# al8n/serf

Hardware: NVIDIA H100
Metric: gossip edge-updates/sec @10M nodes (higher is better)
Workload: dtype u32

## Files before the change

serf_b200/csrc/serfsim.cu:

```cuda
#include <algorithm>
#include <cmath>
#include <cstdio>
#include <cstdlib>
#include <cstring>
#include <string>
#include <unordered_set>
#include <vector>

#include "../../include/serfsim.h"
#include "tick_kernel.cuh"
#include "wire.cuh"

using namespace sfs;

namespace {

thread_local std::string g_err;

int fail(int code, const std::string& msg) { g_err = msg; return code; }

#define CU(call)                                                                              \
  do {                                                                                        \
    cudaError_t e_ = (call);                                                                  \
    if (e_ != cudaSuccess)                                                                    \
// ... 130 lines not shown
  u64* d_grow = nullptr;
  bool gate_on = false;
  u32 gate_first = 0;
  std::vector<u32> launch_log;
  u32 launch_log_first = 0;
  cudaStream_t stream = nullptr;
  cudaEvent_t ev0 = nullptr, ev1 = nullptr;
  bool timing_open = false;
  double last_ms = 0.0;
  u64 last_launches = 0, launches = 0;
  serfsim_event_cb cb = nullptr;
  void* cb_user = nullptr;
  std::vector<u8> reported;
  int grid = 1;
  int ctas_per_sm = 4;
  u64* d_win_data[2] = {nullptr, nullptr};
  u32* d_ctrl = nullptr;
  u32* d_send_count = nullptr;
  u64** d_peer_data[2] = {nullptr, nullptr};
  u32** d_peer_ctrl = nullptr;
  u32 xepoch = 0;
  u32 win_cap = 0;
  u32 win_cap_base = 0;
  bool connected = false;
  bool loopback = false;
  serfsim_barrier_fn barrier = nullptr; serfsim_allreduce_u64_fn allreduce = nullptr; void* comm_user = nullptr;
  std::vector<void*> ipc_opened;
  bool tick_timing = false;
  size_t l2_persist_max = 0, l2_window_max = 0;
  bool l2_window = false;
  bool no_skip = false;
  bool compact = true;
  bool dedup = true;
  struct ResBuf { unsigned char* d = nullptr; cudaEvent_t copied = nullptr; bool used = false; };
  ResBuf res[4];
  u32 res_next = 0;
  cudaStream_t copy_stream = nullptr;
  cudaEvent_t ev_extracted = nullptr;
  std::vector<cudaEvent_t> tick_ev;
  std::vector<cudaEvent_t> mid_ev;
};

namespace {

int slot_of(const serfsim* h, u32 node) {
  for (u32 s = 0; s < h->R; ++s) if (h->subj[s] == node) return (int)s;
  return -1;
}

int ensure_trace(serfsim* h, u32 need) {
  if (need <= h->trace_cap) return 0;
  u32 cap = std::max<u32>(1024, h->trace_cap);
  while (cap < need) cap *= 2;
  u64* nt = nullptr; u32* nk = nullptr; u64* ng = nullptr;
  const bool sharded = h->cfg.world_size > 1;
  CU(cudaMalloc(&nt, (size_t)cap * 8 * sizeof(u64)));
  CU(cudaMalloc(&nk, ((size_t)cap + 1) * 4 * sizeof(u32)));
  CU(cudaMemsetAsync(nt, 0, (size_t)cap * 8 * sizeof(u64), h->stream));
  CU(cudaMemsetAsync(nk, 0, ((size_t)cap + 1) * 4 * sizeof(u32), h->stream));
  if (sharded) { CU(cudaMalloc(&ng, (size_t)cap * 8 * sizeof(u64))); CU(cudaMemsetAsync(ng, 0, (size_t)cap * 8 * sizeof(u64), h->stream)); }
  if (h->d_trace) {
    CU(cudaMemcpyAsync(nt, h->d_trace, (size_t)h->trace_cap * 8 * sizeof(u64), cudaMemcpyDeviceToDevice, h->stream));
    CU(cudaMemcpyAsync(nk, h->d_kinds, ((size_t)h->trace_cap + 1) * 4 * sizeof(u32), cudaMemcpyDeviceToDevice, h->stream));
    if (sharded) CU(cudaMemcpyAsync(ng, h->d_grow, (size_t)h->trace_cap * 8 * sizeof(u64), cudaMemcpyDeviceToDevice, h->stream));
    CU(cudaStreamSynchronize(h->stream));
    cudaFree(h->d_trace); cudaFree(h->d_kinds); cudaFree(h->d_grow);
// ... 43 lines not shown
    const u32 t = h->tick;
    const u64 launches_before = h->last_launches;
    auto lo = std::lower_bound(h->ops.begin(), h->ops.end(), t, [](const HostOp& o, u32 tt) { return o.tick < tt; });
    auto hi = std::upper_bound(h->ops.begin(), h->ops.end(), t, [](u32 tt, const HostOp& o) { return tt < o.tick; });
    const u32 eb = (u32)(lo - h->ops.begin()), ee = (u32)(hi - h->ops.begin());
    for (auto it = lo; it != hi; ++it) {
      const int s = slot_of(h, it->node);
      if (s >= 0) { if (it->op == SERFSIM_OP_FAIL) h->up_mask &= ~(1u << s); if (it->op == SERFSIM_OP_REJOIN) h->up_mask |= (1u << s); }
    }
    if (ee > eb) { launch_mark_events(h->d_busy, h->d_hot[(t & 1) ^ 1], h->d_ev_node, eb, ee, h->first, h->count, h->stream); h->last_launches++; }
    TickParams p{};
    p.n_local = h->count; p.first = h->first; p.n_global = h->N; p.R = h->R;
    p.fanout = h->cfg.fanout; p.probe_every = h->cfg.probe_interval_ticks; p.tick = t;
    p.down_mask = (~h->up_mask) & ((1u << h->R) - 1);
    h->ever_down |= p.down_mask;
    p.seed_lo = (u32)h->cfg.seed; p.seed_hi = (u32)(h->cfg.seed >> 32); p.ev_begin = eb; p.ev_end = ee;
    p.rules = h->rules;
    for (u32 s = 0; s < h->R; ++s) p.subj[s] = h->subj[s];
    p.rec = h->d_rec; p.qword = h->d_qword; p.inbox_rd = h->d_inbox[(t & 1) ^ 1]; p.inbox_wr = h->d_inbox[t & 1];
    p.node_state = h->d_node; p.busy = h->d_busy; p.watch = h->d_watch; p.row_ptr = h->d_rowptr; p.col = h->d_col;
    p.ev_node = h->d_ev_node; p.ev_op = h->d_ev_op; p.ev_slot = h->d_ev_slot;
    p.row = h->d_trace + (size_t)t * 8;
    p.kinds_prev = h->d_kinds + (size_t)t * 4;
    p.kinds_cur = h->d_kinds + ((size_t)t + 1) * 4;
    p.overflow = h->d_overflow;
    p.hot_rd = h->d_hot[(t & 1) ^ 1]; p.hot_wr = h->d_hot[t & 1];
    p.stage_col_bytes = h->stage_col_bytes;
    p.reap_now = (h->cfg.reap_interval_ticks && ((t + 1) % h->cfg.reap_interval_ticks) == 0) ? 1u : 0u;
    p.tombstone_ticks = h->cfg.tombstone_timeout_ticks; p.reconnect_ticks = h->cfg.reconnect_timeout_ticks; p.intent_ticks = h->cfg.recent_intent_timeout_ticks;
    p.stride = h->stride; p.n_tiles = h->n_tiles; p.tiles_per_cta = (h->n_tiles + h->grid - 1) / h->grid;
    p.force_all = (h->cfg.trace != 0) || h->no_skip || p.reap_now;
    p.compact = h->compact ? 1u : 0u;
    p.dedup = h->dedup ? 1u : 0u;
    p.udeg = h->udeg; p.ahead = h->ahead;
    p.tile_due = h->d_tile_due; p.node_due = h->d_node_due; p.hot_static = h->d_hot_static; p.sched = h->d_sched;
    p.sleep_on = (h->no_skip || h->byz_on) ? 0u : 1u;
    p.pp_every = (u32)std::max(0, h->cfg.push_pull_interval_ticks); p.reap_every = h->cfg.reap_interval_ticks;
    p.host_idle_until = h->d_pin_ctl + 2;
    const u32 xpar = h->xepoch & 1;
    p.world = (u32)h->cfg.world_size; p.rank = (u32)h->cfg.rank; p.shard_size = h->shard_size; p.win_cap = h->win_cap;
    p.win_data = h->d_peer_data[xpar]; p.send_count = h->d_send_count;
    p.peer_ctrl = h->d_peer_ctrl; p.stamp = h->xepoch + 1; p.xpar = xpar; p.loopback = h->loopback ? 1u : 0u;
    p.fuse_publish = (sharded && !h->byz_on && !getenv("SERFSIM_NO_FUSE")) ? 1u : 0u;
    p.shard_inv = (u32)(0x100000000ull / h->shard_size); p.xcap = p.world > 1 ? 392u / (p.world - 1) : 0u;
    Gate gate{};
    if (h->gate_on) {
      gate.ctl = h->d_runctl; gate.host_ctl = h->d_pin_ctl; gate.prev_row = t > h->gate_first ? grow + (size_t)(t - 1) * 8 : nullptr; gate.tick = t;
      gate.future_ops = (t > 0 && future_ops(h, t - 1)) ? 1u : 0u;
      gate.pp = (u32)std::max(0, h->cfg.push_pull_interval_ticks); gate.byz_on = h->byz_on ? 1u : 0u;
    }
    const u32* gate_word = h->gate_on ? h->d_runctl : nullptr;
    p.gate = gate; p.gate.evaluate = h->ue_table.n ? 0u : 1u;
    if (h->tick_timing) {
      while (h->tick_ev.size() < 2 * ((size_t)t + 1)) { cudaEvent_t e; CU(cudaEventCreate(&e)); h->tick_ev.push_back(e); }
      CU(cudaEventRecord(h->tick_ev[2 * (size_t)t], h->stream));
    }
    if (h->l2_window && h->l2_window_max) {
      cudaStreamAttrValue av{};
      const size_t bytes = (size_t)3 * h->R * h->stride * sizeof(u32);
      av.accessPolicyWindow.base_ptr = h->d_inbox[t & 1];
      av.accessPolicyWindow.num_bytes = std::min(bytes, h->l2_window_max);
      av.accessPolicyWindow.hitRatio = (float)std::min(1.0, (double)h->l2_persist_max / (double)std::max<size_t>(1, av.accessPolicyWindow.num_bytes));
      av.accessPolicyWindow.hitProp = cudaAccessPropertyPersisting;
      av.accessPolicyWindow.missProp = cudaAccessPropertyStreaming;
      CU(cudaStreamSetAttribute(h->stream, cudaStreamAttributeAccessPolicyWindow, &av));
    }
// ... 394 lines not shown
  CUB(cudaMalloc(&h->d_subj, MAX_SLOTS * 4)); CUB(cudaMalloc(&h->d_scratch, 64 * 8));
  CUB(cudaMalloc(&h->d_stage, (size_t)h->count * 8));
  CUB(cudaMalloc(&h->d_runctl, 2 * sizeof(u32)));
  CUB(cudaMemset(h->d_runctl, 0, 2 * sizeof(u32)));
  CUB(cudaHostAlloc(&h->pin_ctl, 4 * sizeof(u32), cudaHostAllocMapped));
  CUB(cudaHostGetDevicePointer(&h->d_pin_ctl, h->pin_ctl, 0));
  h->pin_ctl[0] = h->pin_ctl[1] = h->pin_ctl[2] = h->pin_ctl[3] = 0;
  CUB(cudaMalloc(&h->d_ones, 16));
  const u32 ones[4] = {0x40000000u, 0x40000000u, 0x40000000u, 1u};
  CUB(cudaMemcpy(h->d_ones, ones, 16, cudaMemcpyHostToDevice));
  CUB(cudaMemcpy(h->d_subj, h->subj.data(), h->R * 4, cudaMemcpyHostToDevice));
  {
    const char* e = getenv("SERFSIM_MINB");
    h->ctas_per_sm = (h->R == 1) ? ((e && atoi(e) == 5) ? 5 : (cfg->world_size > 1 ? tick_ctas_per_sm_r1s() : tick_ctas_per_sm_r1())) : tick_ctas_per_sm_rn();
  }
  h->grid = tick_grid_size(h->count, h->ctas_per_sm);
  h->grid_sv = tick_grid_size(h->count, cfg->world_size > 1 ? tick_ctas_per_sm_r1s() : tick_ctas_per_sm_r1());
  {
    int max_persist = 0, max_window = 0;
    cudaDeviceGetAttribute(&max_persist, cudaDevAttrMaxPersistingL2CacheSize, dev);
    cudaDeviceGetAttribute(&max_window, cudaDevAttrMaxAccessPolicyWindowSize, dev);
    h->l2_persist_max = (size_t)max_persist; h->l2_window_max = (size_t)max_window;
    int want = 0;
    if (const char* e = getenv("SERFSIM_L2_PERSIST")) want = atoi(e);
    if (want && max_persist > 0) cudaDeviceSetLimit(cudaLimitPersistingL2CacheSize, (size_t)max_persist);
    if (const char* e = getenv("SERFSIM_L2_WINDOW")) h->l2_window = atoi(e) != 0;
    if (getenv("SERFSIM_VERBOSE")) fprintf(stderr, "serfsim: L2 persisting max %d B, window max %d B, persist %d window %d\n", max_persist, max_window, want, (int)h->l2_window);
  }
  if (const char* e = getenv("SERFSIM_NO_SKIP")) h->no_skip = atoi(e) != 0;
  if (const char* e = getenv("SERFSIM_COMPACT")) h->compact = atoi(e) != 0;
  if (const char* e = getenv("SERFSIM_DEDUP")) h->dedup = atoi(e) != 0;
  if (const char* e = getenv("SERFSIM_AHEAD")) h->ahead = (u32)std::min(2, std::max(0, atoi(e)));
  if (const char* e = getenv("SERFSIM_SV")) h->sv = (u32)std::min(2, std::max(0, atoi(e)));
  if (cfg->world_size > 1) {
    if (cfg->world_size > 8) return bail(fail(SERFSIM_E_INVAL, "world_size > 8"));
    double factor = 1.25;
    if (const char* e = getenv("SERFSIM_WIN_FACTOR")) factor = atof(e);
    const double pad = (double)std::max(tick_grid_size(h->count, h->ctas_per_sm), h->grid_sv) * 8.0 * 160.0;
    double cap = (double)h->shard_size * cfg->fanout * h->R * 3.0 * factor / cfg->world_size + 4096.0 + pad;
    h->win_cap = (u32)std::min(cap, 4.0e9);
    h->win_cap_base = h->win_cap;
    for (int par = 0; par < 2; ++par) {
      CUB(cudaMalloc(&h->d_win_data[par], (size_t)cfg->world_size * h->win_cap * 8));
      CUB(cudaMemset(h->d_win_data[par], 0, (size_t)cfg->world_size * h->win_cap * 8));
      CUB(cudaMalloc(&h->d_peer_data[par], sizeof(u64*) * 8));
    }
    CUB(cudaMalloc(&h->d_ctrl, CTRL_BYTES));
    CUB(cudaMemset(h->d_ctrl, 0, CTRL_BYTES));
    CUB(cudaMalloc(&h->d_send_count, 8 * sizeof(u32)));
    CUB(cudaMemset(h->d_send_count, 0, 8 * sizeof(u32)));
    CUB(cudaMalloc(&h->d_peer_ctrl, sizeof(u32*) * 8));
    CUB(cudaMalloc(&h->d_anomaly, h->stride)); CUB(cudaMemset(h->d_anomaly, 0, h->stride));
    CUB(cudaMalloc(&h->d_byz_totals, 4 * 8)); CUB(cudaMemset(h->d_byz_totals, 0, 4 * 8));
    CUB(cudaMalloc(&h->d_peer_anomaly, sizeof(void*) * 8));
    if (cfg->push_pull_interval_ticks > 0) {
      CUB(cudaMalloc(&h->d_snap_rec, (size_t)h->R * h->stride * 32));
      CUB(cudaMalloc(&h->d_snap_node, (size_t)h->stride * 8));
      CUB(cudaMalloc(&h->d_peer_snap_rec, sizeof(void*) * 8));
      CUB(cudaMalloc(&h->d_peer_snap_node, sizeof(void*) * 8));
    }
  }
  {
    int rc = ensure_trace(h, 1024);
    if (rc) return bail(rc);
    rc = do_reset(h, cfg->seed);
    if (rc) return bail(rc);
// ... 652 lines not shown
```

serf_b200/csrc/tick_kernel.cu:

```cuda
#include <cstdlib>

#include "tick_kernel.cuh"
#include "byz.cuh"

namespace sfs {

namespace {

constexpr int BLOCK = 256;
#ifndef SFS_MB_R1
#define SFS_MB_R1 3
#endif
#ifndef SFS_MB_R1S
#define SFS_MB_R1S SFS_MB_R1
#endif
#ifndef SFS_MB_RN
#define SFS_MB_RN 1
#endif
constexpr u32 TILE_SHIFT = 8;
constexpr u32 MAX_TILES_PER_CTA = 1024;
static_assert((1u << TILE_SHIFT) == BLOCK, "tile = block");

struct Words { u32 w[8]; };

// ... 2 lines not shown
__device__ __forceinline__ u64 policy_evict_last() { u64 p; asm volatile("createpolicy.fractional.L2::evict_last.b64 %0, 1.0;" : "=l"(p)); return p; }

__device__ __forceinline__ Words ld_rec256(const uint4* ptr, u64 pol) {
  Words r;
  asm volatile("ld.global.L1::no_allocate.L2::cache_hint.v4.u32 {%0,%1,%2,%3}, [%8], %9;\n\t"
               "ld.global.L1::no_allocate.L2::cache_hint.v4.u32 {%4,%5,%6,%7}, [%8+16], %9;"
               : "=r"(r.w[0]), "=r"(r.w[1]), "=r"(r.w[2]), "=r"(r.w[3]), "=r"(r.w[4]), "=r"(r.w[5]), "=r"(r.w[6]), "=r"(r.w[7])
               : "l"(ptr), "l"(pol));
  return r;
}
__device__ __forceinline__ void st_rec256(uint4* ptr, const Words& r, u64 pol) {
  asm volatile("st.global.L2::cache_hint.v4.u32 [%0], {%1,%2,%3,%4}, %9;\n\t"
               "st.global.L2::cache_hint.v4.u32 [%0+16], {%5,%6,%7,%8}, %9;"
               :: "l"(ptr), "r"(r.w[0]), "r"(r.w[1]), "r"(r.w[2]), "r"(r.w[3]), "r"(r.w[4]), "r"(r.w[5]), "r"(r.w[6]), "r"(r.w[7]), "l"(pol) : "memory");
}
__device__ __forceinline__ u64 ld_u64_stream(const u64* ptr, u64 pol) {
  u64 v; asm volatile("ld.global.L1::no_allocate.L2::cache_hint.u64 %0, [%1], %2;" : "=l"(v) : "l"(ptr), "l"(pol)); return v;
}
__device__ __forceinline__ u32 ld_u32_stream(const u32* ptr, u64 pol) {
  u32 v; asm volatile("ld.global.L1::no_allocate.L2::cache_hint.u32 %0, [%1], %2;" : "=r"(v) : "l"(ptr), "l"(pol)); return v;
}
__device__ __forceinline__ void st_u32_stream(u32* ptr, u32 v, u64 pol) {
  asm volatile("st.global.L2::cache_hint.u32 [%0], %1, %2;" :: "l"(ptr), "r"(v), "l"(pol) : "memory");
}
__device__ __forceinline__ void st_u64_stream(u64* ptr, u64 v, u64 pol) {
  asm volatile("st.global.L2::cache_hint.u64 [%0], %1, %2;" :: "l"(ptr), "l"(v), "l"(pol) : "memory");
}
__device__ __forceinline__ void red_max_resident(u32* ptr, u32 v, u64 pol) {
  asm volatile("red.relaxed.gpu.global.max.L2::cache_hint.u32 [%0], %1, %2;" :: "l"(ptr), "r"(v), "l"(pol) : "memory");
}
__device__ __forceinline__ u32 peek_inbox(const u32* ptr, u64 pol) {
  u32 v; asm volatile("ld.global.L1::no_allocate.L2::cache_hint.u32 %0, [%1], %2;" : "=r"(v) : "l"(ptr), "l"(pol)); return v;
}
__device__ __forceinline__ void st_release_sys(u32* ptr, u32 v) { asm volatile("st.release.sys.global.u32 [%0], %1;" :: "l"(ptr), "r"(v) : "memory"); }
__device__ __forceinline__ u32 ld_acquire_sys(const u32* ptr) { u32 f; asm volatile("ld.acquire.sys.global.u32 %0, [%1];" : "=r"(f) : "l"(ptr) : "memory"); return f; }
#else
inline u64 policy_evict_first() { return 0; }
inline u64 policy_evict_last() { return 0; }
inline Words ld_rec256(const uint4* ptr, u64) { emu::probes[8] += 32; Words r; const u32* q = reinterpret_cast<const u32*>(ptr); for (int i = 0; i < 8; ++i) r.w[i] = q[i]; return r; }
inline void st_rec256(uint4* ptr, const Words& r, u64) { emu::probes[9] += 32; u32* q = reinterpret_cast<u32*>(ptr); for (int i = 0; i < 8; ++i) q[i] = r.w[i]; }
inline u64 ld_u64_stream(const u64* ptr, u64) { emu::probes[10] += 8; return *ptr; }
inline u32 ld_u32_stream(const u32* ptr, u64) { emu::probes[11] += 4; return *ptr; }
inline void st_u32_stream(u32* ptr, u32 v, u64) { emu::probes[12] += 4; *ptr = v; }
inline void st_u64_stream(u64* ptr, u64 v, u64) { emu::probes[13] += 8; *ptr = v; }
inline void red_max_resident(u32* ptr, u32 v, u64) { emu::probes[14] += 4; if (v > *ptr) *ptr = v; }
inline u32 peek_inbox(const u32* ptr, u64) { emu::probes[11] += 4; return *ptr; }
inline void st_release_sys(u32* ptr, u32 v) { __atomic_store_n(ptr, v, __ATOMIC_RELEASE); }
inline u32 ld_acquire_sys(const u32* ptr) {
  static thread_local const u32* last = nullptr;
  static thread_local unsigned long spins = 0;
  if (ptr != last) { last = ptr; spins = 0; }
  if (++spins > 64) emu::polite_wait(spins);
  return __atomic_load_n(ptr, __ATOMIC_ACQUIRE);
}
#endif

#ifndef SERFSIM_EMU
__device__ __forceinline__ u32 smem_u32(const void* p) { return (u32)__cvta_generic_to_shared(p); }
__device__ __forceinline__ void mbar_init(u64* bar, u32 count) { asm volatile("mbarrier.init.shared::cta.b64 [%0], %1;" :: "r"(smem_u32(bar)), "r"(count) : "memory"); }
__device__ __forceinline__ void mbar_arrive_expect_tx(u64* bar, u32 bytes) {
  asm volatile("mbarrier.arrive.expect_tx.shared::cta.b64 _, [%0], %1;" :: "r"(smem_u32(bar)), "r"(bytes) : "memory");
}
__device__ __forceinline__ void mbar_arrive(u64* bar) { asm volatile("mbarrier.arrive.shared::cta.b64 _, [%0];" :: "r"(smem_u32(bar)) : "memory"); }
__device__ __forceinline__ void mbar_wait(u64* bar, u32 parity) {
  u32 ok;
  do {
    asm volatile("{\n\t.reg .pred p;\n\tmbarrier.try_wait.parity.shared::cta.b64 p, [%1], %2;\n\tselp.u32 %0, 1, 0, p;\n\t}" : "=r"(ok) : "r"(smem_u32(bar)), "r"(parity) : "memory");
  } while (!ok);
}
__device__ __forceinline__ void fence_proxy_async() { asm volatile("fence.proxy.async.shared::cta;" ::: "memory"); }
__device__ __forceinline__ void bulk_g2s(void* dst, const void* src, u32 bytes, u64* bar, u64 pol) {
  asm volatile("cp.async.bulk.shared::cluster.global.mbarrier::complete_tx::bytes.L2::cache_hint [%0], [%1], %2, [%3], %4;"
               :: "r"(smem_u32(dst)), "l"(src), "r"(bytes), "r"(smem_u32(bar)), "l"(pol) : "memory");
}
#endif

constexpr u32 ST_REC = 0, ST_NODE = 8192, ST_INL = 10240, ST_INJ = 11264, ST_INM = 12288, ST_RP = 13312, ST_COL = 14400;
constexpr u32 RP_BYTES = 1040;
struct StageView {
// ... 152 lines not shown
  u32 srt[FMAX];
#pragma unroll
  for (int k = 0; k < FMAX; ++k) srt[k] = NO_TARGET;
#pragma unroll
  for (int k = 0; k < FMAX; ++k) {
    u32 j = (draw16(w, k) * (deg - min((u32)k, deg))) >> 16;
#pragma unroll
    for (int i = 0; i < k; ++i) j += (j >= srt[i]) ? 1u : 0u;
    const bool use = (u32)k < m;
    const u32 e = row0 + (use ? j : 0u);
    cand[k] = use ? ((STAGED && sv.col_staged) ? sv.col[e - sv.col_base] : SFS_LD_COL(p.col + e, pol_first)) : v;
    u32 x = use ? j : NO_TARGET;
#pragma unroll
    for (int i = 0; i < k; ++i) { const u32 lo = min(srt[i], x), hi = max(srt[i], x); srt[i] = lo; x = hi; }
    srt[k] = x;
  }
}
template <int FMAX>
__device__ __forceinline__ u32 pick_finish(u32 v, const u32 (&cand)[FMAX], u32 (&tg)[FMAX]) {
  u32 nt = 0;
#pragma unroll
  for (int k = 0; k < FMAX; ++k) tg[k] = NO_TARGET;
#pragma unroll
  for (int k = 0; k < FMAX; ++k) {
    if (cand[k] != v) {
#pragma unroll
      for (int j2 = 0; j2 <= k; ++j2) tg[j2] = ((u32)j2 == nt) ? cand[k] : tg[j2];
      ++nt;
    }
  }
  return nt;
}

struct Pre { u32 busy, mL, mJ, mM, any, qw, mailmask, qmask, keep, nd; };
__device__ __forceinline__ u32 carry_of(const TickParams& p, u32 vl) {
  const u32 w = p.carry[vl];
  return (w >> 8) == ((p.tick + 1u) & (CARRY_TICKS - 1u)) ? (w & 0xffu) : 0u;
}
template <bool R1, bool PASS = false>
__device__ __forceinline__ Pre prefetch_node(const TickParams& p, u32 vl, bool kL, bool kJ, bool kM, u64 pol_first, bool due, u32 keep = 0) {
  const u32 nl = p.stride, R = p.R, s_hi = R1 ? 1u : R;
  Pre x;
  x.busy = p.busy[vl];
  x.nd = (!R1 && due) ? p.node_due[vl] : NO_DEADLINE;
  x.keep = R1 ? 0u : keep;
  x.mL = x.mJ = x.mM = x.qw = 0; x.any = 0; x.mailmask = 0; x.qmask = 0;
  for (u32 s2 = 0; s2 < s_hi; ++s2) {
    const u32 l = kL ? ld_u32_stream(p.inbox_rd + (size_t)(KIND_LEAVE * R + s2) * nl + vl, pol_first) : 0u;
    const u32 j = kJ ? ld_u32_stream(p.inbox_rd + (size_t)(KIND_JOIN * R + s2) * nl + vl, pol_first) : 0u;
    const u32 m = kM ? ld_u32_stream(p.inbox_rd + (size_t)(KIND_ML * R + s2) * nl + vl, pol_first) : 0u;
    const u32 q = p.qword[(size_t)s2 * nl + vl];
    SFS_COUNT(6, 4);
    if (R1 || s2 == x.keep) { x.mL = l; x.mJ = j; x.mM = m; x.qw = q; }
    x.any |= l | j | m;
    x.mailmask |= ((l | j | m) ? 1u : 0u) << s2;
    x.qmask |= (q ? 1u : 0u) << s2;
  }
  if (PASS) x.any |= x.qw | ((due && (carry_of(p, vl) & CARRY_TDUE)) ? 1u : 0u);
  return x;
}
__device__ __forceinline__ bool node_active(const TickParams& p, const Pre& x, bool due) {
  return (x.busy & 7u) != 0 || x.any != 0 || p.reap_now != 0 || (due && (x.busy & 8u) && x.nd <= p.tick);
}

template <int FMAX>
struct Ahead { u64 ns; Words rec; u32 cand[FMAX]; u32 valid; };
// ... 41 lines not shown
  return 0;
}
__device__ SFS_COLD void cold_reap(Rec& r, u32 t, u32 tombstone, u32 reconnect, u32 intent) {
  const u32 age = r.leave_tick ? (t + 1 - r.leave_tick) : 0;
  if ((r.flags & 1) && r.leave_tick && ((r.status == ST_LEFT && age > tombstone) || (r.status == ST_FAILED && age > reconnect))) {
    r.flags &= ~1u; r.status = TY_NONE; r.st = 0; r.leave_tick = 0;
  } else if (!(r.flags & 1) && r.status != TY_NONE && r.leave_tick && age > intent) {
    r.status = TY_NONE; r.st = 0; r.leave_tick = 0;
  }
}
__device__ SFS_COLD u32 cold_probe_target(const TickParams& p, u32 v, u32 row0, u32 deg) {
  u32 w[4];
  philox4x32_10(p.tick, v, 0, DOMAIN_PROBE, p.seed_lo, p.seed_hi, w);
  return __ldg(p.col + row0 + (((w[0] & 0xffffu) * deg) >> 16));
}
__device__ SFS_COLD void cold_probe_hit(const TickParams& p, Rec& r, u32 v) {
  if (r.mlstate == ML_ALIVE || r.mlstate == ML_SUSPECT) {
    if (r.mlstate == ML_ALIVE) atomicAdd((unsigned long long*)(p.row + 6), 1ull);
    ml_suspect(r, r.inc, from_bucket(v), p.tick, false, p.rules);
  }
}
__device__ SFS_COLD void cold_refute(Rec& r, u32& clock, u32 limit) {
  const u32 T = clock; witness(clock, T);
  join_intent(r, T, limit);
  r.qjoin = T; r.txj = limit;
}
__device__ SFS_COLD bool cold_can_confirm(u32 k, u32 mask, u32 v) {
  return (u32)__popc(mask) - 1u < k && !(mask & (1u << from_bucket(v)));
}

template <bool TRACE, int FMAX, bool SHARDED, bool R1, bool STAGED, bool PASS = false>
__device__ __forceinline__ bool process_node(const TickParams& p, const StageView& sv, XStage* xs, const u32 vl, const Pre& pre, const bool kL, const bool kJ, const bool kM, const bool mark, const bool saturated,
                                             const bool due, const u64 pol_first, const u64 pol_last, Counters& c, u32& mind, int& dsusp, const Ahead<FMAX>& ah, u32& first_view, const u32 sv_views = 0xffffffffu,
                                             const bool carry_out = false) {
  static_assert(!STAGED || R1, "the staged path is the single-slot path");
  static_assert(!PASS || (R1 && !STAGED && !SHARDED && !TRACE), "passes are single-slot kernels of unsharded production runs");
  const u32 lt = threadIdx.x;
  const u32 v = p.first + vl;
  const u32 t = p.tick;
  const u32 limit = p.rules.limit;
  const u32 nl = p.stride;
  const u32 R = p.R;

  const bool upfront = R1 && (saturated || TRACE || STAGED);
  u64 ns = 0;
  u32 row0 = 0, row1 = 0;
  Words cur;
  auto load_node = [&]() {
    ns = STAGED ? sv.node[lt] : ld_u64_stream(p.node_state + vl, pol_first);
    if (STAGED) { row0 = sv.rowptr[lt]; row1 = sv.rowptr[lt + 1]; }
    else if (p.udeg) { row0 = vl * p.udeg; row1 = row0 + p.udeg; }
    else { row0 = __ldg(p.row_ptr + vl); row1 = __ldg(p.row_ptr + vl + 1); }
  };
  auto load_rec0 = [&]() {
    if (STAGED) {
      const uint4 a = reinterpret_cast<const uint4*>(sv.rec + lt)[0], b = reinterpret_cast<const uint4*>(sv.rec + lt)[1];
      cur.w[0] = a.x; cur.w[1] = a.y; cur.w[2] = a.z; cur.w[3] = a.w; cur.w[4] = b.x; cur.w[5] = b.y; cur.w[6] = b.z; cur.w[7] = b.w;
    } else {
      cur = ld_rec256(p.rec + 2 * (size_t)vl, pol_first);
    }
    merge_q(cur, pre.qw);
  };
  if (upfront) { load_node(); load_rec0(); }
  const u32 busy = pre.busy;
  u32 mL = pre.mL, mJ = pre.mJ, mM = pre.mM;
  if (STAGED) { mL = kL ? sv.inL[lt] : 0u; mJ = kJ ? sv.inJ[lt] : 0u; mM = kM ? sv.inM[lt] : 0u; }

  u32 nd = pre.nd;
  if (R1 && due && (busy & 8u)) nd = p.node_due[vl];
  const u32 sleeping = (due && (busy & 8u)) ? nd : NO_DEADLINE;
  bool timers_due = sleeping <= p.tick;
  u32 cr = 0;
  if (PASS && due) { cr = carry_of(p, vl); if (cr & CARRY_SEEN) timers_due = (cr & CARRY_TDUE) != 0; }
  if (!TRACE && !STAGED && !((busy & 7u) != 0 || pre.any != 0 || p.reap_now != 0 || timers_due)) { mind = min(mind, sleeping); if (due && (busy & 8u)) SFS_PROBE(20); return false; }
  if (PASS && !due) cr = carry_of(p, vl);
  if (STAGED && !TRACE && !((busy & 7u) || (mL | mJ | mM) || p.reap_now || timers_due)) { mind = min(mind, sleeping); return false; }
#define SFS_WMASK() ((busy & 4u) ? ((u32)p.watch[vl] >> p.sv_wshift) : 0u)
  const bool ahead = !R1 && !STAGED && ah.valid;
  if (ahead) { ns = ah.ns; row0 = vl * p.udeg; row1 = row0 + p.udeg; }
  else if (!upfront) { load_node(); if (R1) load_rec0(); }

  u32 clock = (u32)ns;
  const bool up_r = (ns & NS_UP) != 0;
  u32 sstate = (u32)(ns >> 40) & 3;
  const u32 deg = row1 - row0;

  u32 op = 0, op_slot = 0;
  if (busy & 2) { u32 slot_tmp = 0; op = cold_find_op(p, v, slot_tmp); op_slot = slot_tmp; }
  bool up_s = up_r;
  if (op == OP_FAIL) up_s = false;
  if (op == OP_REJOIN) up_s = true;

  bool have_probe = false;
  u32 ptarget = 0;
  if (up_s && (busy & 4u) && p.probe_every && p.down_mask && ((t + v) % p.probe_every) == 0 && deg) {
    ptarget = (STAGED && sv.col_staged) ? 0u : cold_probe_target(p, v, row0, deg);
// ... 55 lines not shown
    const bool self = (p.subj[s] == v);
    const bool susp_before = up_r && r.mlstate == ML_SUSPECT;
    if (!R1 && p.sv_mode == SV_CHECK && !((sv_views >> s) & 1u) && up_r &&
        ((mL | mJ | mM) || (r.txl | r.txj | r.txm) || r.mlstate == ML_SUSPECT)) *p.overflow = 4;

    if (up_r && (mL | mJ | mM)) {
      if (mM) {
        const u32 key = mM - 1, inc = key >> 6, kind = (key >> 4) & 3, fromb = key & 15;
        if (kind == ML_ALIVE) ml_alive(r, inc, self, limit);
        else if (kind == ML_SUSPECT) ml_suspect(r, inc, fromb, t, self, p.rules);
        else ml_dead(r, inc, kind == ML_LEFT, t, self, limit);
      }
      bool refute = false;
      if (mL) { const u32 key = mL - 1, lt = key >> 1; witness(clock, lt); leave_intent(r, lt, !(key & 1u), self, sstate, refute, limit); }
      if (mJ) { const u32 lt = mJ - 1; witness(clock, lt); join_intent(r, lt, limit); }
      if (refute) { Rec tr = r; u32 ck = clock; cold_refute(tr, ck, limit); r = tr; clock = ck; }
      if (!(r.flags & 1) && r.status != TY_NONE && (r.status != (orig.w[6] & 0xff) || r.st != orig.w[0])) r.leave_tick = t + 1;
      Words mid;
      pack_words(r, mid);
      if (R1) c.cp += differs(mid, orig) ? 1u : 0u; else c.changed += differs(mid, orig) ? 1 : 0;
    }
    if (op) { Rec tr = r; u32 ck = clock, ss = sstate; cold_host_op(tr, ck, ss, op, op_slot == s, self, up_r, limit); r = tr; clock = ck; sstate = ss; }
    if (op && !(r.flags & 1) && r.status != TY_NONE && r.leave_tick == 0) r.leave_tick = t + 1;
    if (up_s) {
      if (p.reap_now) { Rec tr = r; cold_reap(tr, t, p.tombstone_ticks, p.reconnect_ticks, p.intent_ticks); r = tr; }
      if (r.mlstate == ML_SUSPECT && r.deadline != 0 && t >= r.deadline) ml_dead(r, r.inc, false, t, false, limit);
      if (have_probe && !self && ptarget == p.subj[s] && ((p.down_mask >> s) & 1)) { Rec tr = r; cold_probe_hit(p, tr, v); r = tr; }
      const u32 mx = max(r.txl, max(r.txj, r.txm));
      if (mx) {
        if (!have_targets) {
          if (ahead) nt = pick_finish<FMAX>(v, ah.cand, tg);
          else {
            u32 cand[FMAX];
            pick_issue<FMAX, STAGED>(p, sv, v, row0, deg, pol_first, cand);
            nt = pick_finish<FMAX>(v, cand, tg);
          }
          have_targets = true;
        }
        u32* const planeL = p.inbox_wr + (size_t)(KIND_LEAVE * R + s) * nl;
        u32* const planeJ = p.inbox_wr + (size_t)(KIND_JOIN * R + s) * nl;
        u32* const planeM = p.inbox_wr + (size_t)(KIND_ML * R + s) * nl;
        const u32 vL = leave_key(r.qleave, (r.flags & FLAG_QPRUNE) != 0) + 1, vJ = r.qjoin + 1, vM = ml_key(r) + 1;
        const u32 sL = min(r.txl, nt), sJ = min(r.txj, nt), sM = min(r.txm, nt);
        if (!SHARDED) {
          send_deduped<FMAX>(p, planeL, tg, sL, vL, pol_last, mark);
          send_deduped<FMAX>(p, planeJ, tg, sJ, vJ, pol_last, mark);
          send_deduped<FMAX>(p, planeM, tg, sM, vM, pol_last, mark);
        } else {
#pragma unroll
          for (int k = 0; k < FMAX; ++k) {
            if ((u32)k < sL) deliver<SHARDED>(p, xs, planeL, tg[k], KIND_LEAVE, s, vL, pol_last, mark);
            if ((u32)k < sJ) deliver<SHARDED>(p, xs, planeJ, tg[k], KIND_JOIN, s, vJ, pol_last, mark);
            if ((u32)k < sM) deliver<SHARDED>(p, xs, planeM, tg[k], KIND_ML, s, vM, pol_last, mark);
          }
        }
        if (R1) { c.kLJ += sL | (sJ << 16); c.kM += sM; c.pe += min(mx, nt) << 16; }
        else { c.kL += sL; c.kJ += sJ; c.kM += sM; c.edges += min(mx, nt); }
        max_tx = max(max_tx, mx);
        r.txl -= sL; r.txj -= sJ; r.txm -= sM;
      }
      if (self && sstate == SS_LEAVING && r.txl == 0 && r.mlstate == ML_ALIVE) {
        r.mlstate = ML_LEFT; r.qfrom = 0; r.txm = limit; sstate = SS_LEFT;
      }
      const bool queued = (r.txl | r.txj | r.txm) != 0;
      if ((!R1 || PASS) && (queued || mx)) c.views |= 1u << (s + p.sv_slot * PASS);
      const bool watching = (busy & 4u) && p.probe_every && ((p.down_mask >> s) & 1) && !self && ((SFS_WMASK() >> s) & 1);
      const bool suspect = r.mlstate == ML_SUSPECT;
// ... 269 lines not shown
      if (threadIdx.x == 0) { SFS_PROBE(0); if (ng > 1) SFS_PROBE(1); if (na > BLOCK) SFS_PROBE(2); }
      for (u32 b0 = 0; b0 < na; b0 += BLOCK) {
        const u32 e = b0 + threadIdx.x;
        if (e < na) {
          const uint4 a = act_s[e];
          const u32 g = (a.x >> 8) & 0xffu;
          const u32 ti = gt_s[g];
          const u32 vl = ((tile0 + ti) << TILE_SHIFT) + (a.x & 0xffu);
          Pre pre;
          if (R1) {
            pre.busy = (a.x >> 16) & 0xffu; pre.any = (a.x >> 24) & 1u; pre.mL = a.y; pre.mJ = a.z; pre.mM = a.w; pre.keep = 0;
            pre.nd = NO_DEADLINE;
            pre.qw = p.qword[vl];
            pre.mailmask = pre.any ? 1u : 0u; pre.qmask = pre.qw ? 1u : 0u;
            SFS_COUNT(6, 4);
          } else {
            pre = prefetch_node<R1, PASS>(p, vl, kL, kJ, kM, pol_first, (hot_s[ti] & 2u) != 0);
          }
          u32 mind = NO_DEADLINE, fv_unused = 0;
          int dsusp = 0;
          const bool pend = process_node<TRACE, FMAX, SHARDED, R1, false, PASS>(p, StageView{}, xs, vl, pre, kL, kJ, kM, mark, false, (hot_s[ti] & 2u) != 0, pol_first, pol_last, c, mind, dsusp, Ahead<FMAX>{}, fv_unused, sv_views, carry_out);
          if (mark && pend) pend_s[g] = 1;
          if (mind != NO_DEADLINE) atomicMin(p.tile_due + tile0 + ti, mind);
          if (dsusp) atomicAdd(&dsusp_s, dsusp);
        }
        if (SHARDED) wrote_remote |= flush_xwarp(p, xs, false, resv, rlen);
      }
      __syncthreads();
      if (mark && threadIdx.x < ng && pend_s[threadIdx.x]) p.hot_wr[tile0 + gt_s[threadIdx.x]] = 1;
      __syncthreads();
    }
  } else {
  const bool ahead_on = !R1 && p.udeg != 0 && (p.ahead == 2u || (p.ahead == 1u && saturated));
  u32 first_view = 0;
  auto prefetch_tile = [&](u32 ti) -> Pre {
    const u32 vn = ((tile0 + ti) << TILE_SHIFT) + threadIdx.x;
    return vn < p.n_local ? prefetch_node<R1, PASS>(p, vn, kL, kJ, kM, pol_first, (hot_s[ti] & 2u) != 0, first_view) : Pre{};
  };
  auto ahead_tile = [&](u32 ti, u32 keep) -> Ahead<FMAX> {
    Ahead<FMAX> a = {};
    const u32 vn = ((tile0 + ti) << TILE_SHIFT) + threadIdx.x;
    if (!R1 && ahead_on && vn < p.n_local) {
      a.ns = ld_u64_stream(p.node_state + vn, pol_first);
      a.rec = ld_rec256(p.rec + 2 * ((size_t)keep * p.stride + vn), pol_first);
      pick_issue<FMAX, false>(p, StageView{}, p.first + vn, vn * p.udeg, p.udeg, pol_first, a.cand);
      a.valid = 1;
      SFS_PROBE(19);
    }
    return a;
  };
  u32 i = 0;
  while (i < ntile && !hot_s[i]) ++i;
  Pre pre_next = {};
  Ahead<FMAX> ah_next = {};
  if (i < ntile) { pre_next = prefetch_tile(i); ah_next = ahead_tile(i, pre_next.keep); }
  while (i < ntile) {
    const Pre pre = pre_next;
    const Ahead<FMAX> ah = ah_next;
    u32 j = i + 1;
    while (j < ntile && !hot_s[j]) ++j;
    if (j < ntile) { pre_next = prefetch_tile(j); ah_next = ahead_tile(j, pre_next.keep); }
    const u32 vl = ((tile0 + i) << TILE_SHIFT) + threadIdx.x;
    bool pend = false;
    u32 mind = NO_DEADLINE;
    int dsusp = 0;
    if (vl < p.n_local) pend = process_node<TRACE, FMAX, SHARDED, R1, false, PASS>(p, StageView{}, xs, vl, pre, kL, kJ, kM, mark, saturated, (hot_s[i] & 2u) != 0, pol_first, pol_last, c, mind, dsusp, ah, first_view, sv_views, carry_out);
    if (mark && __any_sync(0xffffffffu, pend) && lane == 0) p.hot_wr[tile0 + i] = 1;
    note_timers(p, tile0 + i, mind, dsusp, &dsusp_s);
    if (SHARDED) wrote_remote |= flush_xwarp(p, xs, false, resv, rlen);
    i = j;
  }
  }
  if (SHARDED) {
    wrote_remote |= flush_xwarp(p, xs, true, resv, rlen);
    if (wrote_remote) __threadfence_system();
  }
  __syncthreads();
  finish_tick<TRACE, R1, PASS>(p, c, red, dsusp_s);
}

#ifndef SERFSIM_EMU
template <bool TRACE, int FMAX, bool SHARDED, bool BARSYNC>
__global__ void __launch_bounds__(BLOCK, 3) tick_kernel_tma(const __grid_constant__ TickParams p) {
  extern __shared__ __align__(128) unsigned char stage_mem[];
  __shared__ u8 hot_s[MAX_TILES_PER_CTA];
  __shared__ u16 hot_list[MAX_TILES_PER_CTA];
  __shared__ u32 n_hot_s;
  __shared__ u64 red[8][BLOCK / 32];
  __shared__ __align__(8) u64 full_bar[2], empty_bar[2];
  __shared__ u32 col_base_s[2], col_ok_s[2];
  __shared__ int dsusp_s;
  if (gate_closed(p.gate, blockIdx.x == 0 && threadIdx.x == 0)) return;
  if (tick_is_idle(p.sched, p.tick, p.ev_begin, p.ev_end)) { write_idle_row<TRACE>(p); return; }
  Counters c = {};
  const bool kL = p.kinds_prev[KIND_LEAVE] != 0, kJ = p.kinds_prev[KIND_JOIN] != 0, kM = p.kinds_prev[KIND_ML] != 0;
  const u64 pol_first = policy_evict_first(), pol_last = policy_evict_last();
  const int lane = threadIdx.x & 31;

  const u32 prev_msgs = p.kinds_prev[KIND_LEAVE] + p.kinds_prev[KIND_JOIN] + p.kinds_prev[KIND_ML];
// ... 532 lines not shown
```

serf_b200/csrc/tick_kernel.cuh:

```cuda
#pragma once
#include <cuda_runtime.h>

#include "record.cuh"
#include "uevent.cuh"

#if defined(SERFSIM_EMU) && defined(__CUDACC__)
#error "SERFSIM_EMU is the host-only test build of tests/emu (g++); the product is built by nvcc without it"
#endif
#ifndef SERFSIM_EMU
#define SFS_LAUNCH(grid, block, smem, stream, ...) __VA_ARGS__<<<(grid), (block), (smem), (stream)>>>
constexpr int SFS_SMS = 132;
#else
constexpr int SFS_SMS = 1;
#endif
#ifdef SERFSIM_EMU
#define SFS_PROBE(i) (emu::probes[i]++)
#define SFS_COUNT(i, n) (emu::probes[i] += (n))
#else
#define SFS_PROBE(i) ((void)0)
#define SFS_COUNT(i, n) ((void)0)
#endif

namespace sfs {

// ... 42 lines not shown
  const u32* ev_node;
  const u32* ev_op;
  const u32* ev_slot;
  u64* row;
  const u32* kinds_prev;
  u32* kinds_cur;
  u32* overflow;
  u8* hot_rd;
  u8* hot_wr;
  u32 stage_col_bytes, reap_now, dedup, pad3;
  u32 tombstone_ticks, reconnect_ticks, intent_ticks, pad4;
  u32 n_tiles, tiles_per_cta, force_all, stride;
  u32 world, rank, shard_size, win_cap;
  u64* const* win_data;
  u32* send_count;
  const uint4* const* snap_rec_peer; const u64* const* snap_node_peer;
  UeTable ue_table; uint4* ue_state; const uint4* ue_snap; const uint4* const* ue_snap_peer; const u32* ue_ltime; u64* ue_totals;
  u32 compact;
  Gate gate;
  u32 udeg;
  u32* tile_due;
  u32* node_due;
  const u8* hot_static;
  u32* sched;
  u32 sleep_on;
  u32 pp_every, reap_every;
  u32* const* peer_ctrl; u32 stamp, xpar, loopback, fuse_publish;
  u32 shard_inv, xcap;
  u32 sv_wshift;
  u32 sv_mode, views_host, sv_slot, sv_R;
  u32 ahead;
  u32* host_idle_until;
  u32* carry;
};
constexpr u32 SCHED_TICKET = 0, SCHED_IDLE_UNTIL = 1, SCHED_UE_ACTIVITY = 2, SCHED_AWAKE = 3, SCHED_SUSPECTS = 4 ,
              SCHED_LOCAL_QUIET = 6, SCHED_LOCAL_UNTIL = 7 ,
              SCHED_VIEWS_NEW = 8 , SCHED_VIEWS_NEXT = 9 ,
              SCHED_VIEWS_OLD = 10 , SCHED_VIEWS_FROM = 11, SCHED_WORDS = 12;
constexpr u32 SV_OFF = 0, SV_GENERAL = 1, SV_SINGLE = 2, SV_CHECK = 3, SV_PASS = 4;
constexpr u32 CARRY_PK = 0xfu, CARRY_AWAKE = 0x10u, CARRY_TDUE = 0x20u, CARRY_SEEN = 0x40u, CARRY_TICKS = 1u << 24;
constexpr u32 NO_DEADLINE = 0xffffffffu;
__device__ __forceinline__ bool tick_is_idle(const u32* sched, u32 tick, u32 ev_begin, u32 ev_end) {
  return sched && ev_begin == ev_end && tick < sched[SCHED_IDLE_UNTIL];
}

constexpr u32 CTRL_U32 = 2 * 16;
constexpr u32 CTRL_SUMS_OFF = CTRL_U32 * 4;
constexpr u32 CTRL_FIELDS = 11;
constexpr size_t CTRL_BYTES = CTRL_SUMS_OFF + 2 * 8 * CTRL_FIELDS * sizeof(u64);
struct PublishParams {
  u32 world, rank, stamp, xpar;
  u32* send_count;
  u32* const* peer_ctrl;
  const u64* row;
  const u32* gate;
  const u32* sched;
  u32 loopback;
};

struct DrainParams {
  u32 n_local, stride, R, world, rank, win_cap, stamp, n_tiles;
  const u32* kinds_prev;
  u64* win_data;
  const u32* ctrl;
  u32* inbox_wr;
  u8* hot_wr;
// ... 86 lines not shown
```

Baseline: 20.98 billion.

## Stage per-warp CSR neighbor lists into shared memory via cp.async

When at least half of a warp's nodes draw gossip targets, the warp copies its 32 nodes' contiguous CSR column block into shared memory (reusing act_s) with cp.async, and target picking then reads neighbors from shared memory. This is meant to replace scattered per-lane global loads of adjacency entries with coalesced 16-byte bulk loads. It adds a warp-wide copy and wait per node group, plus pressure on shared memory, and only applies to unsharded single-slot fanout-4 runs with small uniform degree.

```diff
diff --git a/serf_b200/csrc/serfsim.cu b/serf_b200/csrc/serfsim.cu
--- a/serf_b200/csrc/serfsim.cu
+++ b/serf_b200/csrc/serfsim.cu
@@ -186,6 +186,7 @@
   bool no_skip = false;
   bool compact = true;
   bool dedup = true;
+  bool csr_stage = true;
   struct ResBuf { unsigned char* d = nullptr; cudaEvent_t copied = nullptr; bool used = false; };
   ResBuf res[4];
   u32 res_next = 0;
@@ -295,6 +296,7 @@
     p.force_all = (h->cfg.trace != 0) || h->no_skip || p.reap_now;
     p.compact = h->compact ? 1u : 0u;
     p.dedup = h->dedup ? 1u : 0u;
+    p.csr_stage = h->csr_stage ? 1u : 0u;
     p.udeg = h->udeg; p.ahead = h->ahead;
     p.tile_due = h->d_tile_due; p.node_due = h->d_node_due; p.hot_static = h->d_hot_static; p.sched = h->d_sched;
     p.sleep_on = (h->no_skip || h->byz_on) ? 0u : 1u;
@@ -755,6 +757,7 @@
   if (const char* e = getenv("SERFSIM_DEDUP")) h->dedup = atoi(e) != 0;
   if (const char* e = getenv("SERFSIM_AHEAD")) h->ahead = (u32)std::min(2, std::max(0, atoi(e)));
   if (const char* e = getenv("SERFSIM_SV")) h->sv = (u32)std::min(2, std::max(0, atoi(e)));
+  if (const char* e = getenv("SERFSIM_CSR_STAGE")) h->csr_stage = atoi(e) != 0;
   if (cfg->world_size > 1) {
     if (cfg->world_size > 8) return bail(fail(SERFSIM_E_INVAL, "world_size > 8"));
     double factor = 1.25;
diff --git a/serf_b200/csrc/tick_kernel.cu b/serf_b200/csrc/tick_kernel.cu
--- a/serf_b200/csrc/tick_kernel.cu
+++ b/serf_b200/csrc/tick_kernel.cu
@@ -58,6 +58,10 @@
 __device__ __forceinline__ u32 peek_inbox(const u32* ptr, u64 pol) {
   u32 v; asm volatile("ld.global.L1::no_allocate.L2::cache_hint.u32 %0, [%1], %2;" : "=r"(v) : "l"(ptr), "l"(pol)); return v;
 }
+__device__ __forceinline__ void cp_async16(void* dst, const void* src, u64 pol) {
+  asm volatile("cp.async.cg.shared.global.L2::cache_hint [%0], [%1], 16, %2;" :: "r"((u32)__cvta_generic_to_shared(dst)), "l"(src), "l"(pol) : "memory");
+}
+__device__ __forceinline__ void cp_async_wait_all() { asm volatile("cp.async.wait_all;" ::: "memory"); }
 __device__ __forceinline__ void st_release_sys(u32* ptr, u32 v) { asm volatile("st.release.sys.global.u32 [%0], %1;" :: "l"(ptr), "r"(v) : "memory"); }
 __device__ __forceinline__ u32 ld_acquire_sys(const u32* ptr) { u32 f; asm volatile("ld.acquire.sys.global.u32 %0, [%1];" : "=r"(f) : "l"(ptr) : "memory"); return f; }
 #else
@@ -71,6 +75,8 @@
 inline void st_u64_stream(u64* ptr, u64 v, u64) { emu::probes[13] += 8; *ptr = v; }
 inline void red_max_resident(u32* ptr, u32 v, u64) { emu::probes[14] += 4; if (v > *ptr) *ptr = v; }
 inline u32 peek_inbox(const u32* ptr, u64) { emu::probes[11] += 4; return *ptr; }
+inline void cp_async16(void* dst, const void* src, u64) { emu::probes[11] += 16; *reinterpret_cast<uint4*>(dst) = *reinterpret_cast<const uint4*>(src); }
+inline void cp_async_wait_all() {}
 inline void st_release_sys(u32* ptr, u32 v) { __atomic_store_n(ptr, v, __ATOMIC_RELEASE); }
 inline u32 ld_acquire_sys(const u32* ptr) {
   static thread_local const u32* last = nullptr;
@@ -289,6 +295,18 @@
   return nt;
 }
 
+constexpr u32 CSR_STAGE_WORDS = 512;
+constexpr u32 CSR_STAGE_MAX_DEG = CSR_STAGE_WORDS / 32;
+__device__ __forceinline__ void stage_csr(const TickParams& p, u32* csr_w, u32 vl0, u64 pol_first) {
+  const u32 lane = threadIdx.x & 31, n16 = 8u * p.udeg;
+  const uint4* src = reinterpret_cast<const uint4*>(p.col) + (size_t)vl0 * p.udeg / 4u;
+  __syncwarp();
+#pragma unroll
+  for (u32 k = 0; k < CSR_STAGE_MAX_DEG / 4; ++k) if (lane + 32u * k < n16) cp_async16(reinterpret_cast<uint4*>(csr_w) + lane + 32u * k, src + lane + 32u * k, pol_first);
+  cp_async_wait_all();
+  __syncwarp();
+}
+
 struct Pre { u32 busy, mL, mJ, mM, any, qw, mailmask, qmask, keep, nd; };
 __device__ __forceinline__ u32 carry_of(const TickParams& p, u32 vl) {
   const u32 w = p.carry[vl];
@@ -396,7 +414,7 @@
 template <bool TRACE, int FMAX, bool SHARDED, bool R1, bool STAGED, bool PASS = false>
 __device__ __forceinline__ bool process_node(const TickParams& p, const StageView& sv, XStage* xs, const u32 vl, const Pre& pre, const bool kL, const bool kJ, const bool kM, const bool mark, const bool saturated,
                                              const bool due, const u64 pol_first, const u64 pol_last, Counters& c, u32& mind, int& dsusp, const Ahead<FMAX>& ah, u32& first_view, const u32 sv_views = 0xffffffffu,
-                                             const bool carry_out = false) {
+                                             const bool carry_out = false, u32* const csr_w = nullptr) {
   static_assert(!STAGED || R1, "the staged path is the single-slot path");
   static_assert(!PASS || (R1 && !STAGED && !SHARDED && !TRACE), "passes are single-slot kernels of unsharded production runs");
   const u32 lt = threadIdx.x;
@@ -426,6 +444,12 @@
     merge_q(cur, pre.qw);
   };
   if (upfront) { load_node(); load_rec0(); }
+  bool csr_staged = false;
+  constexpr bool CSR_STAGE = !SHARDED && R1 && !STAGED && !PASS && FMAX == 4;
+  if (CSR_STAGE && upfront && csr_w) {
+    const bool draws = (pre.any | pre.qw) != 0;
+    if (__popc(__ballot_sync(0xffffffffu, draws)) >= 16) { stage_csr(p, csr_w, vl & ~31u, pol_first); csr_staged = true; }
+  }
   const u32 busy = pre.busy;
   u32 mL = pre.mL, mJ = pre.mJ, mM = pre.mM;
   if (STAGED) { mL = kL ? sv.inL[lt] : 0u; mJ = kJ ? sv.inJ[lt] : 0u; mM = kM ? sv.inM[lt] : 0u; }
@@ -547,7 +571,9 @@
           if (ahead) nt = pick_finish<FMAX>(v, ah.cand, tg);
           else {
             u32 cand[FMAX];
-            pick_issue<FMAX, STAGED>(p, sv, v, row0, deg, pol_first, cand);
+            StageView cs = sv;
+            if (CSR_STAGE && csr_staged) { cs.col = csr_w; cs.col_base = (vl & ~31u) * p.udeg; cs.col_staged = true; SFS_PROBE(23); }
+            pick_issue<FMAX, STAGED || CSR_STAGE>(p, cs, v, row0, deg, pol_first, cand);
             nt = pick_finish<FMAX>(v, cand, tg);
           }
           have_targets = true;
@@ -883,6 +909,9 @@
     }
   } else {
   const bool ahead_on = !R1 && p.udeg != 0 && (p.ahead == 2u || (p.ahead == 1u && saturated));
+  static_assert(sizeof(act_s) >= (BLOCK / 32) * CSR_STAGE_WORDS * sizeof(u32), "CSR stages fit in act_s");
+  constexpr bool CSR_STAGE = !SHARDED && R1 && !PASS && FMAX == 4;
+  const bool csr_on = CSR_STAGE && (saturated || TRACE) && p.csr_stage && p.udeg != 0 && p.udeg <= CSR_STAGE_MAX_DEG;
   u32 first_view = 0;
   auto prefetch_tile = [&](u32 ti) -> Pre {
     const u32 vn = ((tile0 + ti) << TILE_SHIFT) + threadIdx.x;
@@ -915,7 +944,8 @@
     bool pend = false;
     u32 mind = NO_DEADLINE;
     int dsusp = 0;
-    if (vl < p.n_local) pend = process_node<TRACE, FMAX, SHARDED, R1, false, PASS>(p, StageView{}, xs, vl, pre, kL, kJ, kM, mark, saturated, (hot_s[i] & 2u) != 0, pol_first, pol_last, c, mind, dsusp, ah, first_view, sv_views, carry_out);
+    u32* const csr_w = (csr_on && (vl | 31u) < p.n_local) ? reinterpret_cast<u32*>(act_s) + (threadIdx.x >> 5) * CSR_STAGE_WORDS : nullptr;
+    if (vl < p.n_local) pend = process_node<TRACE, FMAX, SHARDED, R1, false, PASS>(p, StageView{}, xs, vl, pre, kL, kJ, kM, mark, saturated, (hot_s[i] & 2u) != 0, pol_first, pol_last, c, mind, dsusp, ah, first_view, sv_views, carry_out, csr_w);
     if (mark && __any_sync(0xffffffffu, pend) && lane == 0) p.hot_wr[tile0 + i] = 1;
     note_timers(p, tile0 + i, mind, dsusp, &dsusp_s);
     if (SHARDED) wrote_remote |= flush_xwarp(p, xs, false, resv, rlen);
diff --git a/serf_b200/csrc/tick_kernel.cuh b/serf_b200/csrc/tick_kernel.cuh
--- a/serf_b200/csrc/tick_kernel.cuh
+++ b/serf_b200/csrc/tick_kernel.cuh
@@ -98,6 +98,7 @@
   u32 ahead;
   u32* host_idle_until;
   u32* carry;
+  u32 csr_stage;
 };
 constexpr u32 SCHED_TICKET = 0, SCHED_IDLE_UNTIL = 1, SCHED_UE_ACTIVITY = 2, SCHED_AWAKE = 3, SCHED_SUSPECTS = 4 ,
               SCHED_LOCAL_QUIET = 6, SCHED_LOCAL_UNTIL = 7 ,
```

Result: no change. 20.95 billion (median of 6 runs) (-0.1%).
